# giltchcity/orb_slam3_ros

Measured on AMD Instinct MI355X. Metric: frames/sec ORB extract+match (752×480, 1000 kp) at 1/2/4/8 GPU; % HBM roofline, higher is better.
Workload: dtype u8; 1 GPU; EuRoC-MH01-like stereo 752x480 (BASELINE config 2): ORBextractor L+R (nFeatures=1000, scale 1.2, 8 levels, FAST 20/7) + ComputeStereoMatches; width=752, height=480, allgather=False, pipelines=1, parallelism=frame-sharded x1

## Files before the change

### orb_slam3_ros_amd/csrc/orbfe_engine.hip

```cpp
#pragma clang fp contract(off)
#include <hip/hip_runtime.h>

#include <algorithm>
#include <atomic>
#include <cmath>
#include <cstdio>
#include <cstdlib>
#include <cstring>
#include <cstddef>
#include <mutex>
#include <vector>

#include "../../include/orbfe.h"
#include "orbfe_types.h"

#include "orbfe_kernels.hip"

using namespace orbfe;

#define HIPCHK(x)                                                                                 \
    do {                                                                                          \
        hipError_t e_ = (x);                                                                      \
        if (e_ != hipSuccess) {                                                                   \
            fprintf(stderr, "orbfe: HIP error %s at %s:%d\n", hipGetErrorString(e_), __FILE__, __LINE__); \
// ... 850 lines not shown
            float t = 0.f;
            HIPCHK(hipEventElapsedTime(&t, h->ev_ring[r][i], h->ev_ring[r][i + 1]));
            ms[i] += t;
        }
    }
    if (n) for (int i = 0; i < ORBFE_NUM_STAGES; i++) ms[i] /= n;
    h->ev_used = 0;
    return n;
}

int orbfe_set_batch_outputs(orbfe_extractor* h, orbfe_keypoint* d_kps, uint8_t* d_desc, int* d_counts,
                            int cap_images) {
    if (!h) return ORBFE_E_ARG;
    h->ext_kps = (OrbKeyPoint*)d_kps;
    h->ext_desc = d_desc;
    h->ext_counts = d_counts;
    h->ext_cap_images = (d_kps && d_desc && d_counts) ? cap_images : 0;
    return ORBFE_OK;
}

int orbfe_extract(orbfe_extractor* h, const uint8_t* img, int width, int height, int stride, int lap0, int lap1,
                  orbfe_keypoint* kps, uint8_t* desc, int cap, int* n) {
    if (!h || !n) return ORBFE_E_ARG;
    *n = 0;
    if (!img || width <= 0 || height <= 0) return ORBFE_E_EMPTY;
    if (stride < width) return ORBFE_E_ARG;
    std::lock_guard<std::mutex> lk(h->mu);
    int rc = ensure(h, width, height, 1);
    if (rc) return rc;
    hipStream_t s = h->own_stream;
    const size_t bytes = (size_t)width * height;
    if (h->stage_bytes < bytes) {
        if (h->d_stage) HIPCHK(hipFree(h->d_stage));
        HIPCHK(hipMalloc(&h->d_stage, bytes));
        h->stage_bytes = bytes;
    }
    const bool tm = h->timing;
    if (tm && !h->call_ev[0])
        for (auto& e : h->call_ev) HIPCHK(hipEventCreate(&e));
    size_t o_kps, o_desc, o_end;
    out_layout(1, h->g.kp_cap, &o_kps, &o_desc, &o_end);
    const size_t kpb = (size_t)h->g.kp_cap * sizeof(OrbKeyPoint), db = (size_t)h->g.kp_cap * 32;
    const size_t pin_need = std::max(bytes, o_end);
    if (h->pin_bytes < pin_need) {
        if (h->h_pin) HIPCHK(hipHostFree(h->h_pin));
        h->h_pin = nullptr;
        h->pin_bytes = 0;
        HIPCHK(hipHostMalloc((void**)&h->h_pin, pin_need, hipHostMallocMapped | hipHostMallocCoherent));
        h->pin_bytes = pin_need;
    }
    if (stride == width) memcpy(h->h_pin, img, bytes);
    else
        for (int y = 0; y < height; y++) memcpy(h->h_pin + (size_t)y * width, img + (size_t)y * stride, width);
    const uint8_t* ptrs[1] = {h->d_stage};
    const int laps[2] = {lap0, lap1};
    uint8_t* hp = h->h_pin;
    uint8_t* hpd = nullptr;
    if (!h->no_push || !h->no_pull) HIPCHK(hipHostGetDevicePointer((void**)&hpd, hp, 0));
    auto enqueue = [&]() -> int {
        if (tm) HIPCHK(hipEventRecord(h->call_ev[0], s));
        if (!h->no_push) {
            hipLaunchKernelGGL(k_push, dim3((unsigned)((bytes / 16 + 1 + 255) / 256)), dim3(256), 0, s,
                               (const uint8_t*)hpd, h->d_stage, bytes);
            HIPCHK(hipGetLastError());
        } else {
            HIPCHK(hipMemcpyAsync(h->d_stage, h->h_pin, bytes, hipMemcpyHostToDevice, s));
        }
        if (tm) HIPCHK(hipEventRecord(h->call_ev[1], s));
        h->timing = false;
        const int r = run_batch(h, 1, ptrs, width, laps, s, false);
        h->timing = tm;
        if (r) return r;
        if (tm) HIPCHK(hipEventRecord(h->call_ev[2], s));
        if (h->cap_b == 1 && kps && desc && !h->no_pull) {
            const int n0 = (int)(o_end / 16);
            hipLaunchKernelGGL(k_pull2, dim3((n0 + 255) / 256), dim3(256), 0, s, (const orbfe_u32x4*)h->d_out,
                               (orbfe_u32x4*)hpd, n0, (const orbfe_u32x4*)nullptr, (orbfe_u32x4*)nullptr, 0);
            HIPCHK(hipGetLastError());
        } else if (h->cap_b == 1 && kps && desc) {
            HIPCHK(hipMemcpyAsync(hp, h->d_out, o_end, hipMemcpyDeviceToHost, s));
        } else {
            HIPCHK(hipMemcpyAsync(hp, h->last_counts, 8, hipMemcpyDeviceToHost, s));
            if (kps) HIPCHK(hipMemcpyAsync(hp + o_kps, h->last_kps, kpb, hipMemcpyDeviceToHost, s));
            if (desc) HIPCHK(hipMemcpyAsync(hp + o_desc, h->last_desc, db, hipMemcpyDeviceToHost, s));
        }
        if (tm) HIPCHK(hipEventRecord(h->call_ev[3], s));
        return ORBFE_OK;
    };
    rc = enqueue();
    if (rc) return rc;
    HIPCHK(hipStreamSynchronize(s));
    int cnt[2];
    memcpy(cnt, hp, 8);
    *n = cnt[0];
    if (cnt[0] > cap) return ORBFE_E_CAPACITY;
    if (cnt[0] > 0) {
        if (kps) memcpy(kps, hp + o_kps, (size_t)cnt[0] * sizeof(OrbKeyPoint));
        if (desc) memcpy(desc, hp + o_desc, (size_t)cnt[0] * 32);
    }
    if (tm) {
        HIPCHK(hipEventElapsedTime(&h->call_ms[0], h->call_ev[0], h->call_ev[1]));
        HIPCHK(hipEventElapsedTime(&h->call_ms[1], h->call_ev[1], h->call_ev[2]));
        HIPCHK(hipEventElapsedTime(&h->call_ms[2], h->call_ev[2], h->call_ev[3]));
    }
    return cnt[1];
}

int orbfe_get_call_timing(orbfe_extractor* h, float* ms) {
    if (!h || !ms) return ORBFE_E_ARG;
    std::lock_guard<std::mutex> lk(h->mu);
    for (int i = 0; i < 5; i++) ms[i] = h->call_ms[i];
    return h->timing ? 5 : 0;
}

int orbfe_pyramid_level(orbfe_extractor* h, int image, int level, uint8_t* dst, int dst_pitch, int* width,
                        int* height) {
    if (!h || level < 0 || level >= h->nlevels || !h->cap_b || image < 0 || image >= h->last_nimg) return ORBFE_E_ARG;
    std::lock_guard<std::mutex> lk(h->mu);
    const OrbLevel& L = h->g.lv[level];
    if (width) *width = L.w;
    if (height) *height = L.h;
    if (!dst) return ORBFE_OK;
    if (dst_pitch < L.w) return ORBFE_E_CAPACITY;
    HIPCHK(hipStreamSynchronize(h->own_stream));
    HIPCHK(hipDeviceSynchronize());
    const uint8_t* src;
    int sp;
    if (level == 0) { src = h->last_ptrs[image]; sp = h->last_pitch; }
    else { src = h->d_pyr + (size_t)image * h->g.pyr_bytes + L.pyr_off; sp = L.pitch; }
    HIPCHK(hipMemcpy2D(dst, dst_pitch, src, sp, L.w, L.h, hipMemcpyDeviceToHost));
    return ORBFE_OK;
}

int orbfe_stereo_match_batch(orbfe_extractor* left, int lbase, int lstep, orbfe_extractor* right, int rbase,
                             int rstep, int nframes, float bf, float fx, float* d_uright, float* d_depth,
                             int* d_nmatch, void* stream) {
    if (!left || !right || nframes <= 0 || !left->cap_b || !right->cap_b) return ORBFE_E_ARG;
    if (left->W != right->W || left->H != right->H || left->nlevels != right->nlevels ||
        left->nfeatures != right->nfeatures || left->scale_factor_f != right->scale_factor_f)
        return ORBFE_E_ARG;
    if (lbase + (nframes - 1) * lstep >= left->last_nimg || rbase + (nframes - 1) * rstep >= right->last_nimg)
        return ORBFE_E_ARG;
    const OrbGeom& g = left->g;
    StereoSide SL{left->d_ptrs, left->last_pitch, left->d_pyr, g.pyr_bytes, left->last_kps, left->last_desc,
                  left->last_counts, lbase, lstep};
    StereoSide SR{right->d_ptrs, right->last_pitch, right->d_pyr, right->g.pyr_bytes, right->last_kps,
                  right->last_desc, right->last_counts, rbase, rstep};
    int sort_cap = 1;
    while (sort_cap < g.kp_cap) sort_cap <<= 1;
    if (g.height + 2 * ST_ROFF + 1 <= (ST_NT / 64) * 128) sort_cap = (g.kp_cap + 3) & ~3;
    const int lkpb = nframes < kSmallBatch ? kSmallStereoLk : ST_LK;
    StereoArgs sa{bf, fx, g.kp_cap, sort_cap, lkpb};
    const size_t lds = (size_t)g.kp_cap * (32 + sizeof(RightRec)) + (size_t)sort_cap * 4 + (ST_NT / 64) * (512 + 128 * 4) +
                       (size_t)round_up(2 * (g.height + 2 * ST_ROFF), 16);
    if (lds > 160 * 1024 - 64 || g.kp_cap > 65535) return ORBFE_E_ARG;
    hipStream_t s = pick_stream(left, stream);
    std::lock_guard<std::mutex> lk(left->mu_stereo);
    if (left->sdist_frames < nframes || left->sdist_kp < g.kp_cap) {
        if (left->d_sdist) HIPCHK(hipFree(left->d_sdist));
        left->d_sdist = nullptr;
        left->sdist_frames = left->sdist_kp = 0;
        HIPCHK(hipMalloc(&left->d_sdist, (size_t)nframes * g.kp_cap * 4));
        left->sdist_frames = nframes;
        left->sdist_kp = g.kp_cap;
    }
    hipLaunchKernelGGL(k_stereo, dim3((g.kp_cap + lkpb - 1) / lkpb, nframes), dim3(ST_NT), lds, s, g, SL, SR, sa,
                       d_uright, d_depth, left->d_sdist);
    hipLaunchKernelGGL(k_stereo_cut, dim3(nframes), dim3(256), 0, s, g, SL, sa, d_uright, d_depth, left->d_sdist,
                       d_nmatch);
    HIPCHK(hipGetLastError());
    return ORBFE_OK;
}

int orbfe_stereo_match(orbfe_extractor* left, orbfe_extractor* right, float bf, float fx, float* uright,
                       float* depth) {
    if (!left || !right) return ORBFE_E_ARG;
    std::lock_guard<std::mutex> lk(left->mu);
    if (!left->d_st || left->stereo_kp < left->g.kp_cap) {
        if (left->d_st) HIPCHK(hipFree(left->d_st));
        left->d_st = nullptr;
        left->d_uright = left->d_depth = nullptr;
        left->d_nmatch = nullptr;
        left->stereo_kp = 0;
        HIPCHK(hipMalloc(&left->d_st, 16 + (size_t)left->g.kp_cap * 8));
        left->d_nmatch = (int*)left->d_st;
        left->d_uright = (float*)(left->d_st + 16);
        left->d_depth = left->d_uright + left->g.kp_cap;
        left->stereo_kp = left->g.kp_cap;
    }
    HIPCHK(hipStreamSynchronize(right->own_stream));
    hipStream_t s = left->own_stream;
    const bool tm = left->timing && left->call_ev[0];
    if (tm) HIPCHK(hipEventRecord(left->call_ev[4], s));
    int rc = orbfe_stereo_match_batch(left, 0, 1, right, 0, 1, 1, bf, fx, left->d_uright, left->d_depth,
                                      left->d_nmatch, s);
    if (rc) return rc;
    if (tm) HIPCHK(hipEventRecord(left->call_ev[5], s));
    const size_t kc = (size_t)left->stereo_kp;
    const size_t need = 32 + 8 * kc;
    if (left->pin_bytes < need) {
        if (left->h_pin) HIPCHK(hipHostFree(left->h_pin));
        left->h_pin = nullptr;
        left->pin_bytes = 0;
        HIPCHK(hipHostMalloc((void**)&left->h_pin, need, hipHostMallocMapped | hipHostMallocCoherent));
        left->pin_bytes = need;
    }
    uint8_t* hp = left->h_pin;
    HIPCHK(hipMemcpyAsync(hp, left->last_counts, 8, hipMemcpyDeviceToHost, s));
    HIPCHK(hipMemcpyAsync(hp + 16, left->d_st, 16 + 8 * kc, hipMemcpyDeviceToHost, s));
    if (tm) HIPCHK(hipEventRecord(left->call_ev[6], s));
    HIPCHK(hipStreamSynchronize(s));
    int cnt[2], nm = 0;
    memcpy(cnt, hp, 8);
    memcpy(&nm, hp + 16, 4);
    if (cnt[0] > 0) {
        memcpy(uright, hp + 32, (size_t)cnt[0] * 4);
        memcpy(depth, hp + 32 + 4 * kc, (size_t)cnt[0] * 4);
    }
    if (tm) {
        HIPCHK(hipEventElapsedTime(&left->call_ms[3], left->call_ev[4], left->call_ev[5]));
        HIPCHK(hipEventElapsedTime(&left->call_ms[4], left->call_ev[5], left->call_ev[6]));
    }
    return nm;
}

static int frame_pair(orbfe_extractor* left, orbfe_extractor* right, const uint8_t* img_left, const uint8_t* img_right,
                      int width, int height, int stride, bool fisheye, int lap0, int lap1, float bf, float fx,
                      float ratio, orbfe_keypoint* kps_left, uint8_t* desc_left, int cap_left, int* n_left,
                      int* mono_left, orbfe_keypoint* kps_right, uint8_t* desc_right, int cap_right, int* n_right,
                      int* mono_right, void* res_a, void* res_b) {
    if (!left || !right || !n_left || !n_right || !mono_left || !mono_right) return ORBFE_E_ARG;
    *n_left = *n_right = 0;
    *mono_left = *mono_right = -1;
    if (!img_left || !img_right || width <= 0 || height <= 0) return ORBFE_E_EMPTY;
    if (stride < width || !kps_left || !desc_left || !kps_right || !desc_right || !res_a || !res_b) return ORBFE_E_ARG;
    if (left != right && (left->nfeatures != right->nfeatures || left->nlevels != right->nlevels ||
                          left->scale_factor_f != right->scale_factor_f || left->ini_th != right->ini_th ||
                          left->min_th != right->min_th || left->resize_simd_lanes != right->resize_simd_lanes ||
                          left->blur_variant != right->blur_variant))
        return ORBFE_E_ARG;
    orbfe_extractor* h = left;
    std::lock_guard<std::mutex> lk(h->mu);
    int rc = ensure(h, width, height, 2);
    if (rc) return rc;
    hipStream_t s = h->own_stream;
    const size_t bytes = (size_t)width * height;
    if (h->stage_bytes < 2 * bytes) {
        if (h->d_stage) HIPCHK(hipFree(h->d_stage));
        h->d_stage = nullptr;
        h->stage_bytes = 0;
        HIPCHK(hipMalloc(&h->d_stage, 2 * bytes));
        h->stage_bytes = 2 * bytes;
    }
    const int kc = h->g.kp_cap;
    if (!h->d_st || h->stereo_kp < kc) {
        if (h->d_st) HIPCHK(hipFree(h->d_st));
        h->d_st = nullptr;
        h->d_uright = h->d_depth = nullptr;
        h->d_nmatch = nullptr;
        h->stereo_kp = 0;
        HIPCHK(hipMalloc(&h->d_st, (16 + (size_t)kc * 8 + 15) & ~(size_t)15));
        h->d_nmatch = (int*)h->d_st;
        h->d_uright = (float*)(h->d_st + 16);
        h->d_depth = h->d_uright + kc;
        h->stereo_kp = kc;
    }
    size_t o_kps, o_desc, o_end;
    out_layout(2, kc, &o_kps, &o_desc, &o_end);
    const size_t o_st = (o_end + 15) & ~(size_t)15, st_bytes = 16 + (size_t)h->stereo_kp * 8;
    const size_t st16 = (st_bytes + 15) & ~(size_t)15;
    const size_t pin_need = std::max(2 * bytes, o_st + st16);
    if (h->pin_bytes < pin_need) {
        if (h->h_pin) HIPCHK(hipHostFree(h->h_pin));
        h->h_pin = nullptr;
        h->pin_bytes = 0;
        HIPCHK(hipHostMalloc((void**)&h->h_pin, pin_need, hipHostMallocMapped | hipHostMallocCoherent));
        h->pin_bytes = pin_need;
    }
    uint8_t* hp = h->h_pin;
    const uint8_t* src[2] = {img_left, img_right};
    const bool tm = h->timing;
    if (tm && !h->call_ev[0])
        for (auto& e : h->call_ev) HIPCHK(hipEventCreate(&e));
    uint8_t* hpd = nullptr;
    if (!h->no_push) HIPCHK(hipHostGetDevicePointer((void**)&hpd, hp, 0));
    const bool split = !h->no_push && (bytes % 16) == 0;
    for (int i = 0; i < 2; i++) {
        if (stride == width) memcpy(hp + i * bytes, src[i], bytes);
        else
            for (int y = 0; y < height; y++)
                memcpy(hp + i * bytes + (size_t)y * width, src[i] + (size_t)y * stride, width);
        if (split) {
            if (i == 0 && tm) HIPCHK(hipEventRecord(h->call_ev[0], s));
            hipLaunchKernelGGL(k_push, dim3((unsigned)((bytes / 16 + 1 + 255) / 256)), dim3(256), 0, s,
                               (const uint8_t*)hpd + i * bytes, h->d_stage + i * bytes, bytes);
            HIPCHK(hipGetLastError());
        }
    }
    const uint8_t* ptrs[2] = {h->d_stage, h->d_stage + bytes};
    const int laps[4] = {fisheye ? lap0 : 0, fisheye ? lap1 : 0, fisheye ? lap0 : 0, fisheye ? lap1 : 0};
    if (!split) {
        if (tm) HIPCHK(hipEventRecord(h->call_ev[0], s));
        if (!h->no_push) {
            hipLaunchKernelGGL(k_push, dim3((unsigned)((2 * bytes / 16 + 1 + 255) / 256)), dim3(256), 0, s,
                               (const uint8_t*)hpd, h->d_stage, 2 * bytes);
            HIPCHK(hipGetLastError());
        } else {
// ... 214 lines not shown
```

### orb_slam3_ros_amd/csrc/orbfe_kernels.hip

```cpp
#pragma clang fp contract(off)
#include <hip/hip_runtime.h>
#include <float.h>
#include <math.h>
#include <stdint.h>

#include <type_traits>

#include "brief_pattern.h"
#include "glibc_sincosf.h"
#include "orbfe_types.h"
#include "stl_sort.h"

namespace orbfe {

#define SYNC() __syncthreads()
#define WAVE_SYNC()                                               \
    do {                                                          \
        __builtin_amdgcn_fence(__ATOMIC_RELEASE, "workgroup");    \
        __builtin_amdgcn_s_waitcnt(0xc07f);                       \
        __builtin_amdgcn_wave_barrier();                          \
        __builtin_amdgcn_fence(__ATOMIC_ACQUIRE, "workgroup");    \
    } while (0)

__constant__ int c_umax[16] = {15, 15, 15, 15, 14, 14, 14, 13, 13, 12, 11, 10, 9, 8, 6, 3};
// ... 1966 lines not shown
                const uint32_t* rp = (const uint32_t*)(raw + (2 * pr + e) * DP_RAW_S) + gq;
                const uint32_t w0 = rp[0], w1 = rp[1], w2 = rp[2];
                h[e][0] = __builtin_amdgcn_udot4(w1, KHI, __builtin_amdgcn_udot4(w0, KLO, 0u, false), false);
                h[e][1] = __builtin_amdgcn_udot4(w1, K11, __builtin_amdgcn_udot4(w0, K10, 0u, false), false);
                h[e][2] = __builtin_amdgcn_udot4(w2, K22, __builtin_amdgcn_udot4(w1, K21, __builtin_amdgcn_udot4(w0, K20, 0u, false), false), false);
                h[e][3] = __builtin_amdgcn_udot4(w2, K32, __builtin_amdgcn_udot4(w1, K31, __builtin_amdgcn_udot4(w0, K30, 0u, false), false), false);
            }
            const bool last = 2 * pr + 1 >= DP_N;
            uint4 pk;
            pk.x = h[0][0] | (last ? 0u : h[1][0] << 16);
            pk.y = h[0][1] | (last ? 0u : h[1][1] << 16);
            pk.z = h[0][2] | (last ? 0u : h[1][2] << 16);
            pk.w = h[0][3] | (last ? 0u : h[1][3] << 16);
            *(uint4*)(rowp + pr * DP_P_S + 4 * gq) = pk;
        }
    }
    WAVE_SYNC();
    const float factorPI = (float)(M_PI / 180.f);
    const float ang = angle * factorPI;
    const float a = glibc_cosf(ang), bs = glibc_sinf(ang);
    typedef float orbfe_f2 __attribute__((ext_vector_type(2)));
    typedef const __attribute__((address_space(3))) uint32_t* lds_u32p;
    const orbfe_f2 cs = {bs, a}, sn = {a, bs}, sg = {1.0f, -1.0f}, mag = {12582930.0f, 12582930.0f};
    const uint32_t S = 4 * DP_P_S;
    const uint32_t KC = (uint32_t)(uintptr_t)(lds_u32p)rowp - 0xA00000u * S - 4u * 0x4B400000u;
    struct Samp { uint32_t ad, sh; };
    auto sample_at = [&](float px, float py) -> Samp {
        const orbfe_f2 u = orbfe_f2{px, px} * cs;
        const orbfe_f2 v = orbfe_f2{py, py} * sn;
        const orbfe_f2 rc = __builtin_elementwise_fma(v, sg, u) + mag;
        const uint32_t rb = __float_as_uint(rc.x), cb = __float_as_uint(rc.y);
        return Samp{__umul24(rb >> 1, S) + 4u * cb + KC, rb << 1};
    };
    const uint32_t C01 = k0 | (k1 << 16), C23 = k2 | (k3 << 16), C21 = k2 | (k1 << 16), C0 = k0;
    auto blurred_at = [&](Samp sp) -> uint32_t {
        const lds_u32p q = (lds_u32p)(size_t)sp.ad;
        const uint32_t d0 = q[0], d1 = q[DP_P_S], d2 = q[2 * DP_P_S], d3 = q[3 * DP_P_S];
        const uint32_t a0 = __builtin_amdgcn_alignbyte(d1, d0, sp.sh), a1 = __builtin_amdgcn_alignbyte(d2, d1, sp.sh);
        const uint32_t a2 = __builtin_amdgcn_alignbyte(d3, d2, sp.sh), a3 = __builtin_amdgcn_alignbyte(0u, d3, sp.sh);
        uint32_t sum = __builtin_amdgcn_udot2(__builtin_bit_cast(orbfe_ushort2, a0), __builtin_bit_cast(orbfe_ushort2, C01), 32768u, false);
        sum = __builtin_amdgcn_udot2(__builtin_bit_cast(orbfe_ushort2, a1), __builtin_bit_cast(orbfe_ushort2, C23), sum, false);
        sum = __builtin_amdgcn_udot2(__builtin_bit_cast(orbfe_ushort2, a2), __builtin_bit_cast(orbfe_ushort2, C21), sum, false);
        sum = __builtin_amdgcn_udot2(__builtin_bit_cast(orbfe_ushort2, a3), __builtin_bit_cast(orbfe_ushort2, C0), sum, false);
        const uint32_t v = sum >> 16;
        return v > 255u ? 255u : v;
    };
    unsigned long long masks[4];
#pragma unroll
    for (int mm = 0; mm < 4; mm++) {
        const orbfe_half2 p0 = __builtin_bit_cast(orbfe_half2, pat[mm].x), p1 = __builtin_bit_cast(orbfe_half2, pat[mm].y);
        const uint32_t t0 = blurred_at(sample_at((float)p0.x, (float)p0.y));
        const uint32_t t1 = blurred_at(sample_at((float)p1.x, (float)p1.y));
        masks[mm] = __ballot(t0 < t1);
    }
    if (lane < 4) {
        unsigned long long mv = lane == 0 ? masks[0] : lane == 1 ? masks[1] : lane == 2 ? masks[2] : masks[3];
        ((unsigned long long*)(desc + o * 32))[lane] = mv;
    }
    emit_kp(angle);
}

#define DP_KPW 4
#ifndef DP_WAVES
#define DP_WAVES 6
#endif
#define DP_ATTR __attribute__((amdgpu_waves_per_eu(DP_WAVES)))
#define DP_WPB 2
template <int KPW>
__global__ __launch_bounds__(64 * DP_WPB) DP_ATTR void k_describe(const uint8_t* const* imgs, int in_pitch, const uint8_t* pyr,
                                                  int pyr_stride, OrbGeom g, const uint32_t* __restrict__ outkeys,
                                                  const int* __restrict__ lvinfo, const int* __restrict__ ranks,
                                                  OrbKeyPoint* kps, uint8_t* desc, int* counts, BlurKernel bk) {
    __shared__ __attribute__((aligned(16))) uint8_t s_dp[DP_WPB][DP_WAVE_LDS];
    __shared__ uint4 s_icm[31][3];
    for (int i = threadIdx.x; i < 31 * 3; i += blockDim.x)
        (&s_icm[0][0])[i] = ((const uint4*)&c_ic_mask.m[0][0])[i];
    __syncthreads();
    const int wave = __builtin_amdgcn_readfirstlane(threadIdx.x >> 6), lane = lane_id();
    const int lb = xcd_logical(block_linear(), gridDim.x * gridDim.y);
    const int b = lb / gridDim.x;
    const int flat0 = ((lb % gridDim.x) * DP_WPB + wave) * KPW;
    if (flat0 >= g.out_per_img) return;
    uint2 pat[4];
#pragma unroll
    for (int mm = 0; mm < 4; mm++) pat[mm] = ((const uint2*)c_pattern_h.v)[64 * mm + lane];
    uint32_t kv = 0;
    int rv = 0;
    if (lane < KPW && flat0 + lane < g.out_per_img) {
        kv = outkeys[(size_t)b * g.out_per_img + flat0 + lane];
        rv = ranks[(size_t)b * g.out_per_img + flat0 + lane];
    }
    const DescImg di = desc_img(g, lvinfo + (size_t)b * g.nlevels * 4, lane);
    if (flat0 == 0 && lane == 0) { counts[2 * b] = di.ntot; counts[2 * b + 1] = di.mono_tot; }
    uint8_t* raw = s_dp[wave];
    uint32_t* rowp = (uint32_t*)(raw + DP_N * DP_RAW_S);
    int lvl = 0;
    DescSlot cur = desc_slot(imgs, in_pitch, pyr, pyr_stride, g, di, kv, rv, 0, &lvl, b, flat0);
    orbfe_u32x4 pq[3];
    if (cur.valid && cur.interior) desc_load(cur, lane, pq);
#pragma unroll
    for (int j = 0; j < KPW; j++) {
        if (cur.valid) {
            if (cur.interior) {
                desc_stage(raw, lane, pq, cur.sh);
            } else {
                const OrbLevel& L = g.lv[cur.l];
                const int px0 = cur.x - DP_R, py0 = cur.y - DP_R;
                for (int it = lane; it < DP_N * DP_N; it += 64) {
                    const int r = it / DP_N, c = it - r * DP_N;
                    raw[r * DP_RAW_S + c] = cur.im[(size_t)reflect101(py0 + r, L.h) * cur.pitch + reflect101(px0 + c, L.w)];
                }
            }
        }
        WAVE_SYNC();
        DescSlot nxt;
        nxt.valid = 0;
        if (j + 1 < KPW) {
            nxt = desc_slot(imgs, in_pitch, pyr, pyr_stride, g, di, kv, rv, j + 1, &lvl, b, flat0 + j + 1);
            if (nxt.valid && nxt.interior) desc_load(nxt, lane, pq);
        }
        if (cur.valid) describe_one(cur, g, raw, rowp, pat, lane, kps, desc, bk, s_icm);
        WAVE_SYNC();
        cur = nxt;
    }
}
#undef DP_ND

struct StereoArgs {
    float bf, fx;
    int max_kp;
    int sort_cap;
    int lk;
};
struct StereoSide {
    const uint8_t* const* imgs;
    int in_pitch;
    const uint8_t* pyr;
    int pyr_stride;
    const OrbKeyPoint* kps;
    const uint8_t* desc;
    const int* counts;
    int base, step;
};
__device__ __forceinline__ int hamming32(const uint32_t* a, const uint32_t* b) {
    int d = 0;
#pragma unroll
    for (int i = 0; i < 8; i++) d += __popc(a[i] ^ b[i]);
    return d;
}
#define ST_LK 512
#define ST_NT 1024
#define ST_ROFF 32
struct RightRec { float x; int minr, maxr, oct; };
__global__ __launch_bounds__(ST_NT) void k_stereo(OrbGeom g, StereoSide SL, StereoSide SR, StereoArgs sa,
                                                  float* uright, float* depth, int* sdist) {
    extern __shared__ __attribute__((aligned(16))) uint8_t smem_st[];
    __shared__ int s_maxspan;
    __shared__ int s_next;
    const int lb = xcd_logical(block_linear(), gridDim.x * gridDim.y);
    const int f = lb / gridDim.x;
    const int bL = SL.base + f * SL.step, bR = SR.base + f * SR.step;
    const int wave = __builtin_amdgcn_readfirstlane(threadIdx.x >> 6), lane = lane_id();
    const int N = SL.counts[2 * bL], Nr = SR.counts[2 * bR];
    const int i0 = (lb % gridDim.x) * sa.lk;
    if (i0 >= N) return;
    const int nrow = g.height + 2 * ST_ROFF;
    const bool csort = nrow + 1 <= (ST_NT / 64) * 128;
    int P = 1;
    while (P < Nr) P <<= 1;
    if (csort) P = Nr;
    uint32_t* s_descR = (uint32_t*)smem_st;
    RightRec* s_rec = (RightRec*)(s_descR + 8 * sa.max_kp);
    uint32_t* s_key = (uint32_t*)(s_rec + sa.max_kp);
    uint8_t* s_win = (uint8_t*)(s_key + sa.sort_cap) + wave * 512;
    int* s_part = (int*)((uint8_t*)(s_key + sa.sort_cap) + (ST_NT / 64) * 512) + wave * 128;
    const OrbKeyPoint* kR = SR.kps + (size_t)bR * g.kp_cap;
    const OrbKeyPoint* kL = SL.kps + (size_t)bL * g.kp_cap;
    const uint4* dR = (const uint4*)(SR.desc + (size_t)bR * g.kp_cap * 32);
    const uint32_t* dL = (const uint32_t*)(SL.desc + (size_t)bL * g.kp_cap * 32);
    if (threadIdx.x == 0) { s_maxspan = 0; s_next = ST_NT / 64; }
    SYNC();
    for (int i = threadIdx.x; i < Nr * 2; i += blockDim.x) ((uint4*)s_descR)[i] = dR[i];
    int span = 0;
    for (int i = threadIdx.x; i < P; i += blockDim.x) {
        uint32_t key = 0xFFFFFFFFu;
        if (i < Nr) {
            const OrbKeyPoint kp = kR[i];
            const float r = 2.0f * g.lv[kp.octave].scale;
            RightRec rr;
            rr.x = kp.x;
            rr.oct = kp.octave;
            rr.maxr = (int)ceilf(kp.y + r);
            rr.minr = (int)floorf(kp.y - r);
            s_rec[i] = rr;
            span = max(span, rr.maxr - rr.minr);
            key = ((uint32_t)(rr.minr + 1024) << 16) | (uint32_t)i;
        }
        s_key[i] = key;
    }
    atomicMax(&s_maxspan, span);
    SYNC();
    uint16_t* s_rowst = (uint16_t*)((uint8_t*)(s_key + sa.sort_cap) + (ST_NT / 64) * (512 + 128 * 4));
    if (csort) {
        int* s_cnt = (int*)((uint8_t*)(s_key + sa.sort_cap) + (ST_NT / 64) * 512);
        for (int r = threadIdx.x; r <= nrow; r += blockDim.x) s_cnt[r] = 0;
        SYNC();
        for (int i = threadIdx.x; i < Nr; i += blockDim.x)
            atomicAdd(&s_cnt[min(max(s_rec[i].minr + ST_ROFF, 0), nrow - 1)], 1);
        SYNC();
        if (wave == 0) (void)wave_scan_lds(s_cnt, nrow + 1);
        SYNC();
        for (int r = threadIdx.x; r < nrow; r += blockDim.x) s_rowst[r] = (uint16_t)s_cnt[r];
        for (int i = threadIdx.x; i < Nr; i += blockDim.x) {
            const int bin = min(max(s_rec[i].minr + ST_ROFF, 0), nrow - 1);
            s_key[atomicAdd(&s_cnt[bin], 1)] = ((uint32_t)(bin - ST_ROFF + 1024) << 16) | (uint32_t)i;
        }
        SYNC();
    } else {
        for (int k = 2; k <= P; k <<= 1)
            for (int j = k >> 1; j > 0; j >>= 1) {
                for (int i = threadIdx.x; i < P; i += blockDim.x) {
                    const int ixj = i ^ j;
                    if (ixj > i) {
                        const uint32_t a = s_key[i], c = s_key[ixj];
                        if ((a > c) == ((i & k) == 0)) { s_key[i] = c; s_key[ixj] = a; }
                    }
                }
                SYNC();
            }
        for (int r = threadIdx.x; r < nrow; r += blockDim.x) {
            const uint32_t t = (uint32_t)max(r - ST_ROFF + 1024, 0) << 16;
            int lo = 0, hi = Nr;
            while (lo < hi) {
                const int mid = (lo + hi) >> 1;
                if (s_key[mid] < t) lo = mid + 1; else hi = mid;
            }
            s_rowst[r] = (uint16_t)lo;
        }
        SYNC();
    }
    const int maxspan = s_maxspan;
    float* uR_out = uright + (size_t)f * g.kp_cap;
    float* dp_out = depth + (size_t)f * g.kp_cap;
    int* sd_out = sdist + (size_t)f * g.kp_cap;
    const float mb = sa.bf / sa.fx;
    const float minZ = mb, minD = 0.f, maxD = sa.bf / minZ;
    const int iend = min(N, i0 + sa.lk);
    for (int iL = i0 + wave; iL < iend;) {
        float outU = -1.0f, outD = -1.0f;
        int outS = -1;
        const OrbKeyPoint kpL = kL[iL];
        const int levelL = kpL.octave;
        const float vL = kpL.y, uL = kpL.x;
        const int row = (int)vL;
        const float minU = uL - maxD, maxU = uL - minD;
        uint32_t dl[8];
#pragma unroll
        for (int k = 0; k < 8; k++) dl[k] = dL[(size_t)iL * 8 + k];
        int bestKey = 0x7fffffff;
        bool anyCand = false;
        auto lower = [&](uint32_t t) {
            int lo = 0, hi = Nr;
            while (lo < hi) {
                const int mid = (lo + hi) >> 1;
                if (s_key[mid] < t) lo = mid + 1; else hi = mid;
            }
            return lo;
        };
        const bool tab = row - maxspan >= -ST_ROFF && row + 1 < g.height + ST_ROFF;
        const int jlo = tab ? (int)s_rowst[row - maxspan + ST_ROFF] : lower((uint32_t)max(row - maxspan + 1024, 0) << 16);
        const int jhi = tab ? (int)s_rowst[row + 1 + ST_ROFF] : lower((uint32_t)max(row + 1 + 1024, 0) << 16);
        for (int j = jlo + lane; j < jhi; j += 64) {
            const int iR = (int)(s_key[j] & 0xFFFFu);
            const RightRec rr = s_rec[iR];
            if (rr.minr <= row && row <= rr.maxr) {
                anyCand = true;
                if (rr.oct >= levelL - 1 && rr.oct <= levelL + 1 && rr.x >= minU && rr.x <= maxU) {
                    const int dist = hamming32(dl, s_descR + 8 * iR);
                    bestKey = min(bestKey, (dist << 16) | iR);
                }
            }
        }
        bestKey = wave_min_dpp(bestKey);
        const bool cand = __any(anyCand) && !(maxU < 0);
        const int bestDist = bestKey == 0x7fffffff ? 100 : min(100, bestKey >> 16);
        if (cand && bestDist < 75) {
            const int bestIdxR = bestKey & 0xffff;
            const float uR0 = s_rec[bestIdxR].x;
            const float sf = g.lv[levelL].inv_scale;
            const float scaleduL = roundf(kpL.x * sf);
            const float scaledvL = roundf(kpL.y * sf);
            const float scaleduR0 = roundf(uR0 * sf);
            const int w = 5, Lr = 5;
            const float iniu = scaleduR0 + Lr - w;
            const float endu = scaleduR0 + Lr + w + 1;
            const OrbLevel& LV = g.lv[levelL];
            if (!(iniu < 0 || endu >= LV.w)) {
                int pL, pR;
                gptr_u8 IL = level_base(SL.imgs, SL.in_pitch, SL.pyr, SL.pyr_stride, g, bL, levelL, &pL);
                gptr_u8 IR = level_base(SR.imgs, SR.in_pitch, SR.pyr, SR.pyr_stride, g, bR, levelL, &pR);
                const int r0 = (int)(scaledvL - w), c0L = (int)(scaleduL - w), c0R = (int)(scaleduR0 - Lr - w);
                uint32_t* s_wl = (uint32_t*)s_win;
                uint32_t* s_wr = (uint32_t*)s_win + 33;
                if (lane < 22) {
                    const bool left = lane < 11;
                    const int yy = left ? lane : lane - 11;
                    gptr_u8 rp = left ? IL + (size_t)(r0 + yy) * pL + c0L : IR + (size_t)(r0 + yy) * pR + c0R;
                    const uint32_t sh = (uint32_t)((uintptr_t)rp & 3);
                    gptr_u32 ap = (gptr_u32)(rp - sh);
                    uint32_t w[7];
#pragma unroll
                    for (int k = 0; k < 7; k++) w[k] = (left && k >= 4) ? 0u : ap[k];
                    if (left) {
#pragma unroll
                        for (int k = 0; k < 3; k++) {
                            uint32_t o = __builtin_amdgcn_alignbyte(w[k + 1], w[k], sh);
                            if (k == 2) o &= 0x00FFFFFFu;
                            s_wl[yy * 3 + k] = o;
                        }
                    } else {
#pragma unroll
                        for (int k = 0; k < 6; k++) s_wr[yy * 6 + k] = __builtin_amdgcn_alignbyte(w[k + 1], w[k], sh);
                    }
                }
                for (int pidx = lane; pidx < 121; pidx += 64) {
                    const int inc = pidx / 11, yy = pidx - inc * 11;
                    const uint32_t* rr = s_wr + yy * 6 + (inc >> 2);
                    const uint32_t ish = (uint32_t)(inc & 3);
                    const uint32_t r0w = __builtin_amdgcn_alignbyte(rr[1], rr[0], ish);
                    const uint32_t r1w = __builtin_amdgcn_alignbyte(rr[2], rr[1], ish);
                    const uint32_t r2w = __builtin_amdgcn_alignbyte(rr[3], rr[2], ish) & 0x00FFFFFFu;
                    const uint32_t* ll = s_wl + yy * 3;
                    s_part[pidx] = (int)__builtin_amdgcn_sad_u8(
                        ll[2], r2w, __builtin_amdgcn_sad_u8(ll[1], r1w, __builtin_amdgcn_sad_u8(ll[0], r0w, 0u)));
                }
                int dsum = 0;
                if (lane < 11)
                    for (int yy = 0; yy < 11; yy++) dsum += s_part[lane * 11 + yy];
                float dists[11];
                int bestD = 0x7fffffff, bestinc = 0;
#pragma unroll
                for (int k = 0; k < 11; k++) {
                    const float dist = (float)__builtin_amdgcn_readlane(dsum, k);
                    dists[k] = dist;
                    if (dist < (float)bestD) { bestD = (int)dist; bestinc = k - Lr; }
                }
                if (!(bestinc == -Lr || bestinc == Lr)) {
                    const float dist1 = dists[Lr + bestinc - 1], dist2 = dists[Lr + bestinc], dist3 = dists[Lr + bestinc + 1];
                    const float deltaR = (dist1 - dist3) / (2.0f * (dist1 + dist3 - 2.0f * dist2));
                    if (!(deltaR < -1 || deltaR > 1)) {
                        float bestuR = LV.scale * ((float)scaleduR0 + (float)bestinc + deltaR);
                        float disparity = (uL - bestuR);
                        if (disparity >= minD && disparity < maxD) {
                            if (disparity <= 0) { disparity = (float)0.01; bestuR = (float)((double)uL - 0.01); }
                            outD = sa.bf / disparity;
                            outU = bestuR;
                            outS = bestD;
                        }
                    }
                }
            }
        }
        if (lane == 0) { uR_out[iL] = outU; dp_out[iL] = outD; sd_out[iL] = outS; }
        int nx = 0;
        if (lane == 0) nx = atomicAdd(&s_next, 1);
        iL = i0 + __builtin_amdgcn_readfirstlane(nx);
    }
}

__device__ __forceinline__ int block256_excl_scan(int v, int* s_ws, int* total) {
    const int lane = lane_id(), wave = threadIdx.x >> 6;
    const int incl = wave_incl_scan(v);
    if (lane == 63) s_ws[wave] = incl;
    SYNC();
    int off = 0, tot = 0;
#pragma unroll
    for (int w = 0; w < 4; w++) {
        const int t = s_ws[w];
        off += w < wave ? t : 0;
        tot += t;
    }
    *total = tot;
    return off + incl - v;
}
__global__ __launch_bounds__(256) void k_stereo_cut(OrbGeom g, StereoSide SL, StereoArgs sa, float* uright,
                                                    float* depth, const int* sdist, int* nmatch) {
    __shared__ int s_h[256];
    __shared__ int s_ws[4];
    __shared__ int s_sel[2];
    const int f = blockIdx.x, t = threadIdx.x;
    const int bL = SL.base + f * SL.step;
    const int N = SL.counts[2 * bL];
    const int* sd = sdist + (size_t)f * g.kp_cap;
    s_h[t] = 0;
    SYNC();
    for (int i = t; i < N; i += blockDim.x) {
        const int d = sd[i];
        if (d >= 0) atomicAdd(&s_h[min(d, 65535) >> 8], 1);
    }
    SYNC();
    int n;
    {
        const int c = s_h[t];
        const int ex = block256_excl_scan(c, s_ws, &n);
        const int k = n / 2;
        if (ex <= k && k < ex + c) { s_sel[0] = t; s_sel[1] = k - ex; }
    }
    if (t == 0) nmatch[f] = n;
    if (n == 0) return;
    SYNC();
    const int hb = s_sel[0], k2 = s_sel[1];
    s_h[t] = 0;
    SYNC();
    for (int i = t; i < N; i += blockDim.x) {
        const int d = sd[i];
        if (d >= 0 && (min(d, 65535) >> 8) == hb) atomicAdd(&s_h[d & 255], 1);
    }
    SYNC();
    {
        int n2;
        const int c = s_h[t];
        SYNC();
        const int ex = block256_excl_scan(c, s_ws, &n2);
        if (ex <= k2 && k2 < ex + c) s_sel[0] = (hb << 8) | t;
    }
    SYNC();
    const float median = (float)s_sel[0];
    const float thDist = 1.5f * 1.4f * median;
    float* uR = uright + (size_t)f * g.kp_cap;
    float* dp = depth + (size_t)f * g.kp_cap;
    for (int i = t; i < N; i += blockDim.x) {
        const int d = sd[i];
        if (d >= 0 && !((float)d < thDist)) { uR[i] = -1; dp[i] = -1; }
    }
}

}
```

Measured before the change: 157,000 frames/s.

## Restructure stereo matching into two phases with 16-lane groups per keypoint

The stereo kernel used to give each left keypoint a whole 64-lane wave for both the candidate search and the SAD window refinement. Now each keypoint gets a 16-lane group, reduced with row DPP, and descriptors are prefetched one round ahead. Surviving keypoints are compacted into an LDS work list, and a second phase does the window SAD with per-lane row loads and DPP row sums. Results are staged in LDS and written out coalesced, and level parameters are cached in LDS. This aims to raise lane utilization and cut the serial per-keypoint LDS round-trips, at the cost of more LDS, extra block syncs and more registers.

```diff
diff --git a/orb_slam3_ros_amd/csrc/orbfe_engine.hip b/orb_slam3_ros_amd/csrc/orbfe_engine.hip
--- a/orb_slam3_ros_amd/csrc/orbfe_engine.hip
+++ b/orb_slam3_ros_amd/csrc/orbfe_engine.hip
@@ -1026,7 +1026,7 @@
     const int lkpb = nframes < kSmallBatch ? kSmallStereoLk : ST_LK;
     StereoArgs sa{bf, fx, g.kp_cap, sort_cap, lkpb};
     const size_t lds = (size_t)g.kp_cap * (32 + sizeof(RightRec)) + (size_t)sort_cap * 4 + (ST_NT / 64) * (512 + 128 * 4) +
-                       (size_t)round_up(2 * (g.height + 2 * ST_ROFF), 16);
+                       (size_t)round_up(2 * (g.height + 2 * ST_ROFF), 16) + ORBFE_MAX_LEVELS * sizeof(StLevel);
     if (lds > 160 * 1024 - 64 || g.kp_cap > 65535) return ORBFE_E_ARG;
     hipStream_t s = pick_stream(left, stream);
     std::lock_guard<std::mutex> lk(left->mu_stereo);
diff --git a/orb_slam3_ros_amd/csrc/orbfe_kernels.hip b/orb_slam3_ros_amd/csrc/orbfe_kernels.hip
--- a/orb_slam3_ros_amd/csrc/orbfe_kernels.hip
+++ b/orb_slam3_ros_amd/csrc/orbfe_kernels.hip
@@ -2142,11 +2142,28 @@
 #define ST_NT 1024
 #define ST_ROFF 32
 struct RightRec { float x; int minr, maxr, oct; };
+struct StLevel { int pitch, pyr_off, w; float scale, inv_scale; int pad[3]; };
+static_assert(ST_LK * 16 <= (ST_NT / 64) * (512 + 128 * 4), "k_stereo: work list exceeds the sort scratch");
+__device__ __forceinline__ int row16_min_dpp(int v) {
+    v = min(v, __builtin_amdgcn_update_dpp(0x7fffffff, v, 0x111, 0xf, 0xf, false));
+    v = min(v, __builtin_amdgcn_update_dpp(0x7fffffff, v, 0x112, 0xf, 0xf, false));
+    v = min(v, __builtin_amdgcn_update_dpp(0x7fffffff, v, 0x114, 0xf, 0xf, false));
+    v = min(v, __builtin_amdgcn_update_dpp(0x7fffffff, v, 0x118, 0xf, 0xf, false));
+    return v;
+}
+__device__ __forceinline__ uint32_t row16_sum_dpp(uint32_t u) {
+    int v = (int)u;
+    v += __builtin_amdgcn_update_dpp(0, v, 0x111, 0xf, 0xf, false);
+    v += __builtin_amdgcn_update_dpp(0, v, 0x112, 0xf, 0xf, false);
+    v += __builtin_amdgcn_update_dpp(0, v, 0x114, 0xf, 0xf, false);
+    v += __builtin_amdgcn_update_dpp(0, v, 0x118, 0xf, 0xf, false);
+    return (uint32_t)v;
+}
 __global__ __launch_bounds__(ST_NT) void k_stereo(OrbGeom g, StereoSide SL, StereoSide SR, StereoArgs sa,
                                                   float* uright, float* depth, int* sdist) {
     extern __shared__ __attribute__((aligned(16))) uint8_t smem_st[];
     __shared__ int s_maxspan;
-    __shared__ int s_next;
+    __shared__ int s_nitem;
     const int lb = xcd_logical(block_linear(), gridDim.x * gridDim.y);
     const int f = lb / gridDim.x;
     const int bL = SL.base + f * SL.step, bR = SR.base + f * SR.step;
@@ -2162,13 +2179,12 @@
     uint32_t* s_descR = (uint32_t*)smem_st;
     RightRec* s_rec = (RightRec*)(s_descR + 8 * sa.max_kp);
     uint32_t* s_key = (uint32_t*)(s_rec + sa.max_kp);
-    uint8_t* s_win = (uint8_t*)(s_key + sa.sort_cap) + wave * 512;
-    int* s_part = (int*)((uint8_t*)(s_key + sa.sort_cap) + (ST_NT / 64) * 512) + wave * 128;
+    uint8_t* s_scr = (uint8_t*)(s_key + sa.sort_cap);
     const OrbKeyPoint* kR = SR.kps + (size_t)bR * g.kp_cap;
     const OrbKeyPoint* kL = SL.kps + (size_t)bL * g.kp_cap;
     const uint4* dR = (const uint4*)(SR.desc + (size_t)bR * g.kp_cap * 32);
     const uint32_t* dL = (const uint32_t*)(SL.desc + (size_t)bL * g.kp_cap * 32);
-    if (threadIdx.x == 0) { s_maxspan = 0; s_next = ST_NT / 64; }
+    if (threadIdx.x == 0) { s_maxspan = 0; s_nitem = 0; }
     SYNC();
     for (int i = threadIdx.x; i < Nr * 2; i += blockDim.x) ((uint4*)s_descR)[i] = dR[i];
     int span = 0;
@@ -2190,9 +2206,17 @@
     }
     atomicMax(&s_maxspan, span);
     SYNC();
-    uint16_t* s_rowst = (uint16_t*)((uint8_t*)(s_key + sa.sort_cap) + (ST_NT / 64) * (512 + 128 * 4));
+    uint16_t* s_rowst = (uint16_t*)(s_scr + (ST_NT / 64) * (512 + 128 * 4));
+    StLevel* s_lv = (StLevel*)((uint8_t*)s_rowst + ((2 * nrow + 15) & ~15));
+    if (threadIdx.x < ORBFE_MAX_LEVELS) {
+        const OrbLevel& L = g.lv[threadIdx.x];
+        StLevel t;
+        t.pitch = L.pitch; t.pyr_off = L.pyr_off; t.w = L.w; t.scale = L.scale; t.inv_scale = L.inv_scale;
+        t.pad[0] = t.pad[1] = t.pad[2] = 0;
+        s_lv[threadIdx.x] = t;
+    }
     if (csort) {
-        int* s_cnt = (int*)((uint8_t*)(s_key + sa.sort_cap) + (ST_NT / 64) * 512);
+        int* s_cnt = (int*)(s_scr + (ST_NT / 64) * 512);
         for (int r = threadIdx.x; r <= nrow; r += blockDim.x) s_cnt[r] = 0;
         SYNC();
         for (int i = threadIdx.x; i < Nr; i += blockDim.x)
@@ -2230,131 +2254,204 @@
         SYNC();
     }
     const int maxspan = s_maxspan;
-    float* uR_out = uright + (size_t)f * g.kp_cap;
-    float* dp_out = depth + (size_t)f * g.kp_cap;
-    int* sd_out = sdist + (size_t)f * g.kp_cap;
     const float mb = sa.bf / sa.fx;
     const float minZ = mb, minD = 0.f, maxD = sa.bf / minZ;
-    const int iend = min(N, i0 + sa.lk);
-    for (int iL = i0 + wave; iL < iend;) {
-        float outU = -1.0f, outD = -1.0f;
-        int outS = -1;
-        const OrbKeyPoint kpL = kL[iL];
-        const int levelL = kpL.octave;
-        const float vL = kpL.y, uL = kpL.x;
-        const int row = (int)vL;
-        const float minU = uL - maxD, maxU = uL - minD;
-        uint32_t dl[8];
-#pragma unroll
-        for (int k = 0; k < 8; k++) dl[k] = dL[(size_t)iL * 8 + k];
-        int bestKey = 0x7fffffff;
-        bool anyCand = false;
-        auto lower = [&](uint32_t t) {
-            int lo = 0, hi = Nr;
-            while (lo < hi) {
-                const int mid = (lo + hi) >> 1;
-                if (s_key[mid] < t) lo = mid + 1; else hi = mid;
-            }
-            return lo;
-        };
-        const bool tab = row - maxspan >= -ST_ROFF && row + 1 < g.height + ST_ROFF;
-        const int jlo = tab ? (int)s_rowst[row - maxspan + ST_ROFF] : lower((uint32_t)max(row - maxspan + 1024, 0) << 16);
-        const int jhi = tab ? (int)s_rowst[row + 1 + ST_ROFF] : lower((uint32_t)max(row + 1 + 1024, 0) << 16);
-        for (int j = jlo + lane; j < jhi; j += 64) {
-            const int iR = (int)(s_key[j] & 0xFFFFu);
-            const RightRec rr = s_rec[iR];
-            if (rr.minr <= row && row <= rr.maxr) {
-                anyCand = true;
-                if (rr.oct >= levelL - 1 && rr.oct <= levelL + 1 && rr.x >= minU && rr.x <= maxU) {
-                    const int dist = hamming32(dl, s_descR + 8 * iR);
-                    bestKey = min(bestKey, (dist << 16) | iR);
+    const int nk = min(N, i0 + sa.lk) - i0;
+    const int grp = lane >> 4, l16 = lane & 15;
+    const int gid = grp * (ST_NT / 64) + wave;
+    uint4* s_item = (uint4*)s_scr;
+    {
+        const int roundsA = (nk + 63) >> 6;
+        int kn = i0 + min(gid, nk - 1);
+        float nx = kL[kn].x, ny = kL[kn].y;
+        int noct = kL[kn].octave;
+        uint32_t ndl[8];
+#pragma unroll
+        for (int k = 0; k < 8; k++) ndl[k] = dL[(size_t)kn * 8 + k];
+        for (int t = 0; t < roundsA; t++) {
+            const int key = gid + 64 * t;
+            const bool kvalid = key < nk;
+            const float uL = nx, vL = ny;
+            const int levelL = noct;
+            uint32_t dl[8];
+#pragma unroll
+            for (int k = 0; k < 8; k++) dl[k] = ndl[k];
+            kn = i0 + min(key + 64, nk - 1);
+            nx = kL[kn].x;
+            ny = kL[kn].y;
+            noct = kL[kn].octave;
+#pragma unroll
+            for (int k = 0; k < 8; k++) ndl[k] = dL[(size_t)kn * 8 + k];
+            const int row = (int)vL;
+            const float minU = uL - maxD, maxU = uL - minD;
+            int bestKey = 0x7fffffff;
+            bool anyCand = false;
+            auto lower = [&](uint32_t tk) {
+                int lo = 0, hi = Nr;
+                while (lo < hi) {
+                    const int mid = (lo + hi) >> 1;
+                    if (s_key[mid] < tk) lo = mid + 1; else hi = mid;
                 }
-            }
-        }
-        bestKey = wave_min_dpp(bestKey);
-        const bool cand = __any(anyCand) && !(maxU < 0);
-        const int bestDist = bestKey == 0x7fffffff ? 100 : min(100, bestKey >> 16);
-        if (cand && bestDist < 75) {
-            const int bestIdxR = bestKey & 0xffff;
-            const float uR0 = s_rec[bestIdxR].x;
-            const float sf = g.lv[levelL].inv_scale;
-            const float scaleduL = roundf(kpL.x * sf);
-            const float scaledvL = roundf(kpL.y * sf);
-            const float scaleduR0 = roundf(uR0 * sf);
-            const int w = 5, Lr = 5;
-            const float iniu = scaleduR0 + Lr - w;
-            const float endu = scaleduR0 + Lr + w + 1;
-            const OrbLevel& LV = g.lv[levelL];
-            if (!(iniu < 0 || endu >= LV.w)) {
-                int pL, pR;
-                gptr_u8 IL = level_base(SL.imgs, SL.in_pitch, SL.pyr, SL.pyr_stride, g, bL, levelL, &pL);
-                gptr_u8 IR = level_base(SR.imgs, SR.in_pitch, SR.pyr, SR.pyr_stride, g, bR, levelL, &pR);
-                const int r0 = (int)(scaledvL - w), c0L = (int)(scaleduL - w), c0R = (int)(scaleduR0 - Lr - w);
-                uint32_t* s_wl = (uint32_t*)s_win;
-                uint32_t* s_wr = (uint32_t*)s_win + 33;
-                if (lane < 22) {
-                    const bool left = lane < 11;
-                    const int yy = left ? lane : lane - 11;
-                    gptr_u8 rp = left ? IL + (size_t)(r0 + yy) * pL + c0L : IR + (size_t)(r0 + yy) * pR + c0R;
-                    const uint32_t sh = (uint32_t)((uintptr_t)rp & 3);
-                    gptr_u32 ap = (gptr_u32)(rp - sh);
-                    uint32_t w[7];
-#pragma unroll
-                    for (int k = 0; k < 7; k++) w[k] = (left && k >= 4) ? 0u : ap[k];
-                    if (left) {
-#pragma unroll
-                        for (int k = 0; k < 3; k++) {
-                            uint32_t o = __builtin_amdgcn_alignbyte(w[k + 1], w[k], sh);
-                            if (k == 2) o &= 0x00FFFFFFu;
-                            s_wl[yy * 3 + k] = o;
-                        }
-                    } else {
-#pragma unroll
-                        for (int k = 0; k < 6; k++) s_wr[yy * 6 + k] = __builtin_amdgcn_alignbyte(w[k + 1], w[k], sh);
+                return lo;
+            };
+            int jlo = 0, jhi = 0;
+            if (kvalid) {
+                if (row - maxspan >= -ST_ROFF && row + 1 < g.height + ST_ROFF) {
+                    jlo = (int)s_rowst[row - maxspan + ST_ROFF];
+                    jhi = (int)s_rowst[row + 1 + ST_ROFF];
+                } else {
+                    jlo = lower((uint32_t)max(row - maxspan + 1024, 0) << 16);
+                    jhi = lower((uint32_t)max(row + 1 + 1024, 0) << 16);
+                }
+            }
+            for (int j = jlo + l16; j < jhi; j += 16) {
+                const int iR = (int)(s_key[j] & 0xFFFFu);
+                const RightRec rr = s_rec[iR];
+                if (rr.minr <= row && row <= rr.maxr) {
+                    anyCand = true;
+                    if (rr.oct >= levelL - 1 && rr.oct <= levelL + 1 && rr.x >= minU && rr.x <= maxU) {
+                        const int dist = hamming32(dl, s_descR + 8 * iR);
+                        bestKey = min(bestKey, (dist << 16) | iR);
                     }
                 }
-                for (int pidx = lane; pidx < 121; pidx += 64) {
-                    const int inc = pidx / 11, yy = pidx - inc * 11;
-                    const uint32_t* rr = s_wr + yy * 6 + (inc >> 2);
-                    const uint32_t ish = (uint32_t)(inc & 3);
-                    const uint32_t r0w = __builtin_amdgcn_alignbyte(rr[1], rr[0], ish);
-                    const uint32_t r1w = __builtin_amdgcn_alignbyte(rr[2], rr[1], ish);
-                    const uint32_t r2w = __builtin_amdgcn_alignbyte(rr[3], rr[2], ish) & 0x00FFFFFFu;
-                    const uint32_t* ll = s_wl + yy * 3;
-                    s_part[pidx] = (int)__builtin_amdgcn_sad_u8(
-                        ll[2], r2w, __builtin_amdgcn_sad_u8(ll[1], r1w, __builtin_amdgcn_sad_u8(ll[0], r0w, 0u)));
+            }
+            bestKey = row16_min_dpp(bestKey);
+            const bool cand = ((__ballot(anyCand) >> (16 * grp)) & 0xFFFFull) != 0 && !(maxU < 0);
+            const int bestDist = bestKey == 0x7fffffff ? 100 : min(100, bestKey >> 16);
+            bool emit = false;
+            uint4 item = make_uint4(0u, 0u, 0u, 0u);
+            if (l16 == 15 && kvalid && cand && bestDist < 75) {
+                const int bestIdxR = bestKey & 0xffff;
+                const float uR0 = s_rec[bestIdxR].x;
+                const StLevel LV = s_lv[levelL];
+                const float sf = LV.inv_scale;
+                const float scaledvL = roundf(vL * sf);
+                const float scaleduR0 = roundf(uR0 * sf);
+                const int w = 5, Lr = 5;
+                const float iniu = scaleduR0 + Lr - w;
+                const float endu = scaleduR0 + Lr + w + 1;
+                if (!(iniu < 0 || endu >= LV.w)) {
+                    emit = true;
+                    item = make_uint4(__float_as_uint(uL), __float_as_uint(scaleduR0), (uint32_t)(int)(scaledvL - w),
+                                      (uint32_t)key | ((uint32_t)levelL << 16));
                 }
-                int dsum = 0;
-                if (lane < 11)
-                    for (int yy = 0; yy < 11; yy++) dsum += s_part[lane * 11 + yy];
-                float dists[11];
+            }
+            const unsigned long long em = __ballot(emit);
+            if (em) {
+                int base = 0;
+                if (lane == 0) base = atomicAdd(&s_nitem, __popcll(em));
+                base = __builtin_amdgcn_readfirstlane(base);
+                if (emit) s_item[base + lanes_below(em)] = item;
+            }
+        }
+    }
+    SYNC();
+    const int M = s_nitem;
+    float* s_resU = (float*)s_descR;
+    float* s_resD = s_resU + nk;
+    int* s_resS = (int*)(s_resD + nk);
+    for (int i = threadIdx.x; i < nk; i += blockDim.x) { s_resU[i] = -1.0f; s_resD[i] = -1.0f; s_resS[i] = -1; }
+    SYNC();
+    if (M > 0) {
+        const gptr_u8 IL0 = as_global(SL.imgs[bL]), IR0 = as_global(SR.imgs[bR]);
+        const gptr_u8 PL = as_global(SL.pyr + (size_t)bL * SL.pyr_stride), PR = as_global(SR.pyr + (size_t)bR * SR.pyr_stride);
+        const int yy = min(l16, 10);
+        auto fetch = [&](const uint4 it, uint32_t (&wl)[4], uint32_t (&wr)[7]) -> uint32_t {
+            const int lvl = (int)(it.w >> 16);
+            const StLevel LV = s_lv[lvl];
+            const float uL = __uint_as_float(it.x), scaleduR0 = __uint_as_float(it.y);
+            const int w = 5, Lr = 5;
+            const float scaleduL = roundf(uL * LV.inv_scale);
+            const int r0 = (int)it.z, c0L = (int)(scaleduL - w), c0R = (int)(scaleduR0 - Lr - w);
+            const int pL = lvl == 0 ? SL.in_pitch : LV.pitch, pR = lvl == 0 ? SR.in_pitch : LV.pitch;
+            const gptr_u8 IL = lvl == 0 ? IL0 : PL + LV.pyr_off;
+            const gptr_u8 IR = lvl == 0 ? IR0 : PR + LV.pyr_off;
+            const gptr_u8 rl = IL + (size_t)(r0 + yy) * pL + c0L;
+            const gptr_u8 rr = IR + (size_t)(r0 + yy) * pR + c0R;
+            const uint32_t shl = (uint32_t)((uintptr_t)rl & 3), shr = (uint32_t)((uintptr_t)rr & 3);
+            const gptr_u32 al = (gptr_u32)(rl - shl), ar = (gptr_u32)(rr - shr);
+#pragma unroll
+            for (int k = 0; k < 4; k++) wl[k] = al[k];
+#pragma unroll
+            for (int k = 0; k < 7; k++) wr[k] = ar[k];
+            return shl | (shr << 2);
+        };
+        const int roundsB = (M + 63) >> 6;
+        uint4 nit = s_item[min(gid, M - 1)];
+        uint32_t nwl[4], nwr[7];
+        uint32_t nsh = fetch(nit, nwl, nwr);
+        for (int t = 0; t < roundsB; t++) {
+            const int idx = gid + 64 * t;
+            const uint4 it = nit;
+            const uint32_t shl = nsh & 3u, shr = nsh >> 2;
+            uint32_t wl[4], wr[7];
+#pragma unroll
+            for (int k = 0; k < 4; k++) wl[k] = nwl[k];
+#pragma unroll
+            for (int k = 0; k < 7; k++) wr[k] = nwr[k];
+            nit = s_item[min(idx + 64, M - 1)];
+            nsh = fetch(nit, nwl, nwr);
+            uint32_t ll[3], rw[6];
+#pragma unroll
+            for (int k = 0; k < 3; k++) ll[k] = __builtin_amdgcn_alignbyte(wl[k + 1], wl[k], shl);
+            ll[2] &= 0x00FFFFFFu;
+#pragma unroll
+            for (int k = 0; k < 6; k++) rw[k] = __builtin_amdgcn_alignbyte(wr[k + 1], wr[k], shr);
+            const bool rowlane = l16 < 11;
+            uint32_t dsum[11];
+#pragma unroll
+            for (int inc = 0; inc < 11; inc++) {
+                const int q = inc >> 2;
+                const uint32_t ish = (uint32_t)(inc & 3);
+                const uint32_t r0w = __builtin_amdgcn_alignbyte(rw[q + 1], rw[q], ish);
+                const uint32_t r1w = __builtin_amdgcn_alignbyte(rw[q + 2], rw[q + 1], ish);
+                const uint32_t r2w = __builtin_amdgcn_alignbyte(q + 3 < 6 ? rw[q + 3] : 0u, rw[q + 2], ish) & 0x00FFFFFFu;
+                const uint32_t sad = __builtin_amdgcn_sad_u8(
+                    ll[2], r2w, __builtin_amdgcn_sad_u8(ll[1], r1w, __builtin_amdgcn_sad_u8(ll[0], r0w, 0u)));
+                dsum[inc] = row16_sum_dpp(rowlane ? sad : 0u);
+            }
+            if (l16 == 15 && idx < M) {
+                const int Lr = 5;
+                const int lvl = (int)(it.w >> 16), key = (int)(it.w & 0xFFFFu);
+                const float uL = __uint_as_float(it.x), scaleduR0 = __uint_as_float(it.y);
+                const float scale = s_lv[lvl].scale;
+                float dist1 = 0.f, dist2 = 0.f, dist3 = 0.f;
                 int bestD = 0x7fffffff, bestinc = 0;
 #pragma unroll
                 for (int k = 0; k < 11; k++) {
-                    const float dist = (float)__builtin_amdgcn_readlane(dsum, k);
-                    dists[k] = dist;
-                    if (dist < (float)bestD) { bestD = (int)dist; bestinc = k - Lr; }
+                    const float dist = (float)(int)dsum[k];
+                    if (dist < (float)bestD) {
+                        bestD = (int)dist;
+                        bestinc = k - Lr;
+                        dist1 = k > 0 ? (float)(int)dsum[k > 0 ? k - 1 : 0] : 0.f;
+                        dist2 = dist;
+                        dist3 = k < 10 ? (float)(int)dsum[k < 10 ? k + 1 : 10] : 0.f;
+                    }
                 }
                 if (!(bestinc == -Lr || bestinc == Lr)) {
-                    const float dist1 = dists[Lr + bestinc - 1], dist2 = dists[Lr + bestinc], dist3 = dists[Lr + bestinc + 1];
                     const float deltaR = (dist1 - dist3) / (2.0f * (dist1 + dist3 - 2.0f * dist2));
                     if (!(deltaR < -1 || deltaR > 1)) {
-                        float bestuR = LV.scale * ((float)scaleduR0 + (float)bestinc + deltaR);
+                        float bestuR = scale * ((float)scaleduR0 + (float)bestinc + deltaR);
                         float disparity = (uL - bestuR);
                         if (disparity >= minD && disparity < maxD) {
                             if (disparity <= 0) { disparity = (float)0.01; bestuR = (float)((double)uL - 0.01); }
-                            outD = sa.bf / disparity;
-                            outU = bestuR;
-                            outS = bestD;
+                            s_resD[key] = sa.bf / disparity;
+                            s_resU[key] = bestuR;
+                            s_resS[key] = bestD;
                         }
                     }
                 }
             }
         }
-        if (lane == 0) { uR_out[iL] = outU; dp_out[iL] = outD; sd_out[iL] = outS; }
-        int nx = 0;
-        if (lane == 0) nx = atomicAdd(&s_next, 1);
-        iL = i0 + __builtin_amdgcn_readfirstlane(nx);
+    }
+    SYNC();
+    float* uR_out = uright + (size_t)f * g.kp_cap + i0;
+    float* dp_out = depth + (size_t)f * g.kp_cap + i0;
+    int* sd_out = sdist + (size_t)f * g.kp_cap + i0;
+    for (int i = threadIdx.x; i < nk; i += blockDim.x) {
+        uR_out[i] = s_resU[i];
+        dp_out[i] = s_resD[i];
+        sd_out[i] = s_resS[i];
     }
 }
 
```

After: 158,800 frames/s (median of 6 runs). 1.01x the previous value.
